# AnnSeidel/genometools

Hardware: AMD Instinct MI355X
Metric: Gbp/s ESA build (suf+lcp+bwt), 3 Gbp DNA, 1/2/4/8 MI355X; bit-exact vs CPU (higher is better)
Workload: dtype u64; 1 GPU; human-like DNA (2% N, 24 seqs, repeats) n=3000000000 seed=43 -suf -lcp -bwt (BASELINE.json configs[2]); parallelism=1 device, pair_suffixes=341032298, tied_suffixes=390540711, refine_rounds=9, maxbranchdepth=8256

## Files before the change

### genometools_amd/csrc/esa_engine.hip

```cpp
#include <stdarg.h>
#include <stdlib.h>
#include <chrono>
#include <type_traits>
#include <utility>
#include <vector>
#include "../../include/gtamd_esa.h"
#include "esa_prims.h"
#include "esa_devutil.h"
#include "esa_own.h"

static thread_local char g_err[1024] = "";
void gtamd_set_error(const char *fmt, ...) {
  va_list ap;
  va_start(ap, fmt);
  vsnprintf(g_err, sizeof g_err, fmt, ap);
  va_end(ap);
}
extern "C" const char *gtamd_esa_last_error(void) { return g_err; }

extern "C" int gtamd_device_count(void) {
  GTAMD_ABI_BEGIN
  int n = 0;
  if (hipGetDeviceCount(&n) != hipSuccess) return 0;
  return n;
// ... 2443 lines not shown
    const long v = atol(e);
    if (v >= MS_TILE && v <= (long) MSD_BIG_MAX) sw.msd_big_max = (u32) v;
  }
  sw.msd_radix = flag("GTAMD_MSD_RADIX", '1');
  if (const char *e = getenv("GTAMD_MSD_PACK")) sw.msd_pack = atoi(e) != 0;
  if (const char *e = getenv("GTAMD_MSD_PACK_CAP")) {
    const long v = atol(e);
    if (v >= 1024 && v <= (long) MD_CAP) sw.msd_pack_cap = (u32) v;
  }
  if (const char *e = getenv("GTAMD_MSD_BIN_LIMIT")) {
    const long v = atol(e);
    if (v >= 2 && v <= 4096) sw.msd_bin_limit = (u32) v;
  }
  sw.fused_pass0 = !flag("GTAMD_FUSED_PASS0", '0');
  sw.force_wide = flag("GTAMD_FORCE_WIDE", '1');
  sw.no_pairs = flag("GTAMD_NO_PAIRS", '1');
  sw.no_small_groups = flag("GTAMD_NO_SMALL_GROUPS", '1');
  if (const char *e = getenv("GTAMD_APPLY_EARLY")) sw.apply_early = atoi(e);
  if (sw.apply_early < 0 || sw.apply_early > 2) sw.apply_early = 0;
  if (const char *e = getenv("GTAMD_APPLY_WGS")) {
    const long v = atol(e);
    if (v >= 64 && v <= (1 << 22)) sw.apply_wgs = (u64) v;
    sw.apply_wgs_given = true;
  }
  if (const char *e = getenv("GTAMD_RANK_WINDOW_BITS")) {
    const int v = atoi(e);
    if (v >= 2 && v <= RW_BITS) sw.rank_window_bits = v;
  }
  sw.rank_all_windows = flag("GTAMD_RANK_ALL_WINDOWS", '1');
  sw.win_filter_global = flag("GTAMD_WIN_FILTER_LDS", '0');
  if (const char *e = getenv("GTAMD_PAIR_CHUNK")) {
    const int v = atoi(e);
    if (v >= 4 && v <= 1024) sw.pair_chunk = v;
  }
  if (const char *e = getenv("GTAMD_ROUND_STRIDE")) {
    const int v = atoi(e);
    if (v >= RT_STRIDE_MIN && v <= RT_TILE) sw.round_stride = (u32) v;
  }
  sw.debug = getenv("GTAMD_DEBUG") != nullptr;
  return sw;
}

struct gtamd_esa_ctx {
  int device = 0;
  u32 sigma = 0;
  int bits = 0;
  u64 max_n = 0, n = 0, N = 0;
  int readmode = 0;
  Stream st, st2;
  Event ev_sorted, ev_emitted, ev_applied;
  DevBuf tb_own, sp_own;
  Text text = {};
  bool have_text = false;
  DevBuf k0, k1, v0, v1;
  DevBuf isa_tmp;
  DevBuf rws;
  DevBuf msd;
  DevBuf suf, lcp, bwt;
  DevBuf tiebits, tiebits2;
  DevBuf arena;
  DevBuf arena_p;
  DevBuf xrecv;
  DevBuf winbuf;
  DevBuf lcpfull_buf;
  DevBuf partws;
  DevBuf posw;
  Dev<u64> llv;
  u64 llv_pairs = 0;
  Dev<u32> bck;
  u64 bck_codes = 0, bck_special = 0, bck_dist = 0;
  Dev<Stats> d_stats;
  Pinned<Stats> h_stats;
  Pinned<u32> h_counts;
  Pinned<u32> h_hist;
  u32 user_prefixlength = 0;
  u32 part = 0, numparts = 1;
  gtamd_allgather_fn comm_allgather = nullptr;
  gtamd_alltoallv_fn comm_alltoallv = nullptr;
  void (*comm_abort)(void *) = nullptr;
  void *comm_abort_user = nullptr;
  void *comm_user = nullptr;
  u64 NL = 0, index_offset = 0;
  Dev<u32> d_parthist;
  Dev<u8> d_owner;
  Dev<u32> d_counts;
  u32 want = 0;
  bool ran = false;
  gtamd_esa_stats stats = {};
  gtamd_esa_timing timing = {};
  u64 alloc_bytes = 0;
  float alloc_ms = 0;
  Event ev[8];
  Event ev_scatter[2 * 16];
};

enum TimingEvent {
  EV_START,
  EV_KEYS,
  EV_SORTED,
  EV_TIEBITS,
  EV_REFINE_BEGIN,
  EV_REFINE_END,
  EV_DONE
};

static int ensure_buf(gtamd_esa_ctx *c, DevBuf &b, u64 bytes, const char *what) {
// ... 104 lines not shown
  GTAMD_ABI_BEGIN
  if (c == nullptr) { gtamd_set_error("null context"); return -1; }
  c->comm_allgather = ag;
  c->comm_alltoallv = a2a;
  c->comm_user = user;
  c->comm_abort = nullptr;
  c->comm_abort_user = nullptr;
  return 0;
  GTAMD_ABI_END(-1)
}

extern "C" int gtamd_esa_set_comm_abort(gtamd_esa_ctx *c, void (*abort_fn)(void *), void *user) {
  GTAMD_ABI_BEGIN
  if (c == nullptr) { gtamd_set_error("null context"); return -1; }
  c->comm_abort = abort_fn;
  c->comm_abort_user = user;
  return 0;
  GTAMD_ABI_END(-1)
}

extern "C" int gtamd_esa_set_prefixlength(gtamd_esa_ctx *c, uint32_t k) {
  GTAMD_ABI_BEGIN
  if (c == nullptr) { gtamd_set_error("null context"); return -1; }
  const u32 maxk = c->bits == 2 ? (u32) KeyLayout<2>::KEY_SYMS : (u32) KeyLayout<5>::KEY_SYMS;
  if (k > maxk) {
    gtamd_set_error("prefix length %u is too large: the maximal prefix length "
                    "for this engine is %u", k, maxk);
    return -1;
  }
  c->user_prefixlength = k;
  return 0;
  GTAMD_ABI_END(-1)
}

extern "C" int gtamd_esa_set_readmode(gtamd_esa_ctx *c, int readmode) {
  GTAMD_ABI_BEGIN
  if (c == nullptr) { gtamd_set_error("null context"); return -1; }
  if (readmode < 0 || readmode > 3) {
    gtamd_set_error("invalid readmode %d (0 forward, 1 reverse, 2 complement, "
                    "3 reverse complement)", readmode);
    return -1;
  }
  if (readmode >= 2 && c->sigma != 4) {
    gtamd_set_error("readmode %s is only defined for DNA alphabets",
                    readmode == 2 ? "cpl" : "rcl");
    return -1;
  }
  c->readmode = readmode;
  c->have_text = false;
  return 0;
  GTAMD_ABI_END(-1)
}

static int set_n(gtamd_esa_ctx *c, u64 n) {
  if (n > c->max_n) {
    gtamd_set_error("sequence length %llu exceeds the context capacity %llu",
                    (unsigned long long) n, (unsigned long long) c->max_n);
    return -1;
  }
  c->n = n;
  c->N = n + 1;
  c->ran = false;
  return 0;
}

extern "C" int gtamd_esa_set_sequence_bytes(gtamd_esa_ctx *c,
                                            const uint8_t *enc, uint64_t n,
                                            int is_device) {
  GTAMD_ABI_BEGIN
  if (c == nullptr) { gtamd_set_error("null context"); return -1; }
  TRY(set_n(c, n));
  HIP_TRY(hipSetDevice(c->device));
  const u64 spw = c->bits == 2 ? 32 : 12;
  const u64 nw_tb = div_up(c->N, spw), nw_sp = div_up(c->N, 64);
  TRY(ensure_buf(c, c->tb_own, (nw_tb + 2) * 8, "the packed sequence"));
  TRY(ensure_buf(c, c->sp_own, (nw_sp + 2) * 8, "the special bitmap"));
  const u8 *d_enc = enc;
  Dev<u8> staged;
  if (!is_device && n > 0) {
    HIP_TRY(staged.alloc(n));
    HIP_TRY(hipMemcpyAsync(staged, enc, n, hipMemcpyHostToDevice, c->st));
    d_enc = staged;
  }
  u64 *tb = c->tb_own.as<u64>(), *sp = c->sp_own.as<u64>();
  const int rev = c->readmode & 1, cpl = c->readmode >> 1;
  if (c->bits == 2)
    k_pack_symbols<2><<<(u32) div_up(nw_tb, 256), 256, 0, c->st>>>(d_enc, n, tb, nw_tb, rev, cpl);
  else
    k_pack_symbols<5><<<(u32) div_up(nw_tb, 256), 256, 0, c->st>>>(d_enc, n, tb, nw_tb, rev, cpl);
  HIP_TRY(hipGetLastError());
  k_pack_specials<<<(u32) div_up(nw_sp, 256), 256, 0, c->st>>>(d_enc, n, sp, nw_sp, rev);
  HIP_TRY(hipGetLastError());
  HIP_TRY(hipStreamSynchronize(c->st));
  c->text.tb = tb; c->text.sp = sp; c->text.n = n;
  c->text.nw_tb = nw_tb; c->text.nw_sp = nw_sp;
  c->have_text = true;
  return 0;
  GTAMD_ABI_END(-1)
}

extern "C" int gtamd_esa_set_sequence_packed(gtamd_esa_ctx *c,
                                             const uint64_t *twobit,
                                             const uint64_t *specialbits,
                                             uint64_t n) {
  GTAMD_ABI_BEGIN
  if (c == nullptr) { gtamd_set_error("null context"); return -1; }
  if (c->bits != 2) {
    gtamd_set_error("packed input is defined for the 2-bit DNA layout only");
    return -1;
  }
  if (c->readmode != 0) {
    gtamd_set_error("packed input is read in place: readmode %d cannot be applied "
                    "(hand the sequence in as bytes)", c->readmode);
    return -1;
  }
  TRY(set_n(c, n));
  c->text.tb = twobit; c->text.sp = specialbits; c->text.n = n;
  c->text.nw_tb = div_up(n, 32); c->text.nw_sp = div_up(n + 1, 64);
  c->have_text = true;
  return 0;
  GTAMD_ABI_END(-1)
}

static int fetch_stats(gtamd_esa_ctx *c) {
  HIP_TRY(hipMemcpyAsync(c->h_stats, c->d_stats, sizeof(Stats),
                         hipMemcpyDeviceToHost, c->st));
  HIP_TRY(hipStreamSynchronize(c->st));
  return 0;
}

static int bits_for(u64 maxvalue) {
  int b = 1;
  while (b < 64 && (maxvalue >> b) != 0) b++;
  return b;
}

struct Bump {
  u8 *base;
  u64 off;
  template <typename T> T *take(u64 count) {
    off = (off + 255) & ~255ull;
    T *p = base != nullptr ? reinterpret_cast<T *>(base + off) : nullptr;
    off += count * sizeof(T);
    return p;
  }
};

static int comm_allgather(gtamd_esa_ctx *c, int failed, const void *send, void *recv,
                          u32 bytes) {
  const u32 R = c->numparts;
  if (R == 1 && c->comm_allgather == nullptr) {
    if (bytes) memcpy(recv, send, bytes);
    return failed ? -1 : 0;
  }
  std::vector<u8> mine(8 + (size_t) bytes), all((size_t) R * (8 + bytes));
  const u64 status = failed ? 1 : 0;
  memcpy(mine.data(), &status, 8);
  if (bytes) memcpy(mine.data() + 8, send, bytes);
  const auto t0 = std::chrono::steady_clock::now();
  const int rc = c->comm_allgather(c->comm_user, mine.data(), all.data(), 8 + bytes);
  c->timing.comm_ms += std::chrono::duration<float, std::milli>(
                           std::chrono::steady_clock::now() - t0).count();
  c->timing.comm_calls++;
  if (rc != 0) {
    gtamd_set_error("allgather callback failed");
    return -1;
  }
  int bad = -1;
  for (u32 r = 0; r < R; r++) {
    u64 s;
    memcpy(&s, all.data() + (size_t) r * (8 + bytes), 8);
// ... 78 lines not shown
    k_bck_count<BITS><<<(u32) div_up(NL, 256), 256, 0, st>>>(
        skey, NL, k, c->sigma, c->bck, c->bck + codes + 1,
        c->bck + codes + 1 + special, c->text, spos);
    HIP_TRY(hipGetLastError());
  }
  u32 *ws = c->rws.as<u32>();
  Dev<u32> own;
  if (scan_workspace_words(codes + 1) * 4 > c->rws.bytes) {
    HIP_TRY(own.alloc(scan_workspace_words(codes + 1) * 4));
    ws = own;
  }
  TRY(scan_u32(SCAN_SUM, c->bck, c->bck, codes + 1, false, ws, st));
  c->bck_codes = codes; c->bck_special = special; c->bck_dist = dist;
  return 0;
}

static u64 rws_words_for(u64 cap) {
  return radix_workspace_words(cap) + 10 * (div_up(cap, 64) + 64) +
         scan_workspace_words(div_up(cap, 64)) + 64;
}
static int ensure_workspace(gtamd_esa_ctx *c, u64 cap, u32 want, bool dist) {
  const u64 pad = cap + 8;
  TRY(ensure_buf(c, c->k0, pad * 8, "sort keys"));
  TRY(ensure_buf(c, c->k1, pad * 8, "sort keys"));
  TRY(ensure_buf(c, c->v0, pad * 4, "sort values"));
  TRY(ensure_buf(c, c->v1, pad * 4, "sort values"));
  TRY(ensure_buf(c, c->rws, rws_words_for(cap) * 4, "the radix workspace"));
  TRY(ensure_buf(c, c->tiebits, (div_up(cap, 64) + 2) * 8, "the tie bitmap"));
  if (want & GTAMD_WANT_SUF) TRY(ensure_buf(c, c->suf, pad * 8, "the suffix table"));
  if (want & GTAMD_WANT_LCP) TRY(ensure_buf(c, c->lcp, pad, "the lcp table"));
  if (want & GTAMD_WANT_BWT) TRY(ensure_buf(c, c->bwt, pad, "the bwt table"));
  if (dist) TRY(ensure_buf(c, c->isa_tmp, pad * 8, "the exchange scratch"));
  return 0;
}

static int msd_cbits_max(u64 N) {
  const int c = bits_for(N > 1 ? N - 1 : 1) - 24;
  return c < 0 ? 0 : (c > 8 ? 8 : c);
}
static int msd_choose_cbits(u64 N, int cmax, const float *penalty) {
  int best = cmax;
  float best_cost = 0.0f;
  for (int k = 1; k >= 0; k--) {
    const int c = cmax - 2 + k;
    if (c < 6) continue;
    const float gain = k == 1 ? 0.17f : 0.57f;
    const float cost = (penalty[k] - penalty[2]) / (float) N - gain;
    if (cost < best_cost) { best = c; best_cost = cost; }
  }
  return best;
}
struct MsdWs {
  u32 *hist, *scanws, *tcnt, *tfirst, *dtcnt, *dtfirst, *startA, *startB, *F, *scan2, *counters,
      *biglist, *giantlist, *crowdlist, *bndA;
  MsTile *desc;
  MdTile *dtiles;
  u64 *firstkey, *lastkey;
  u32 rows, tilesB_ub, tilesC_ub, tilesD_ub;
  u64 nf;
};
static u64 msd_carve(u64 N, int cb, u8 *base, MsdWs *w) {
  const u32 ntA = (u32) div_up(N, MS_TILE);
  w->tilesB_ub = ntA + 256;
  w->tilesC_ub = ntA + MSD_PARENTS;
  w->tilesD_ub = (u32) (2 * div_up(N, MS_TILE)) + MSD_PARENTS + 8;
  w->rows = w->tilesC_ub + 2;
  w->nf = (u64) MSD_PARENTS << cb;
  Bump b;
  b.base = base;
  b.off = 0;
  w->hist = b.take<u32>((u64) w->rows * 256);
  w->scanws = b.take<u32>(radix_rows_workspace_words(w->rows));
  w->desc = b.take<MsTile>(w->tilesC_ub);
  w->tcnt = b.take<u32>(MSD_PARENTS + 8);
  w->tfirst = b.take<u32>(MSD_PARENTS + 8);
  w->dtcnt = b.take<u32>(MSD_PARENTS + 8);
  w->dtfirst = b.take<u32>(MSD_PARENTS + 8);
  w->startA = b.take<u32>(256 + 8);
  w->bndA = b.take<u32>(256 * MSD_BLOCKS);
  w->startB = b.take<u32>(MSD_PARENTS + 8);
  w->F = b.take<u32>(w->nf + 8);
  w->scan2 = b.take<u32>(scan_workspace_words(w->nf + 1) + 64);
  w->counters = b.take<u32>(16);
  w->dtiles = b.take<MdTile>(w->tilesD_ub);
  w->firstkey = b.take<u64>(w->tilesD_ub);
  w->lastkey = b.take<u64>(w->tilesD_ub);
  w->biglist = b.take<u32>(w->tilesD_ub);
  w->crowdlist = b.take<u32>(w->tilesD_ub);
  w->giantlist = b.take<u32>((u64) (N / MS_TILE) + 8);
  return b.off + 256;
}

static int msd_level_prepare(gtamd_esa_ctx *c, const MsdWs &w, const u32 *pstart, u32 np, int cb,
                             u32 tiles_ub, const u32 *kin, const u64 *ein, u32 *cstart) {
  hipStream_t st = c->st;
  k_msd_tilecount<<<(np + 1 + 255) / 256, 256, 0, st>>>(pstart, 0, np, (u32) MS_TILE, w.tcnt);
  HIP_TRY(hipGetLastError());
  TRY(scan_u32(SCAN_SUM, w.tcnt, w.tfirst, (u64) np + 1, false, w.scan2, st));
  k_msd_tiledesc<<<(tiles_ub + 255) / 256, 256, 0, st>>>(pstart, w.tfirst, np, tiles_ub, w.desc);
  HIP_TRY(hipGetLastError());
  if (ein != nullptr)
    k_msd_hist_lvl<u64><<<tiles_ub + 1, MS_THREADS, 0, st>>>(ein, w.desc, tiles_ub, 32 - cb, w.hist);
  else
    k_msd_hist_lvl<u32><<<tiles_ub + 1, MS_THREADS, 0, st>>>(kin, w.desc, tiles_ub, 32 - cb, w.hist);
  HIP_TRY(hipGetLastError());
  TRY(radix_scan_tile_rows(w.hist, tiles_ub + 1, w.scanws, st));
  const u64 nchild = (u64) np << cb;
  k_msd_tot<<<(u32) div_up(nchild + 1, 256), 256, 0, st>>>(w.hist, w.tfirst, np, cb, cstart);
  HIP_TRY(hipGetLastError());
  TRY(scan_u32(SCAN_SUM, cstart, cstart, nchild + 1, false, w.scan2, st));
  return 0;
}

struct MsdPartSrc {
  const u64 *ck;
  const u32 *cp32;
  u64 index_offset;
  const unsigned long long *prev_key;
  int has_prev;
};
template <int FMT>
static int msd_sort_emit(gtamd_esa_ctx *c, const Switches &sw, u32 want, u32 prefixlength, u64 N,
                         u64 density_n, const MsdPartSrc *src, u32 **sa_out,
                         u64 **fkey, u32 **fval, u64 *local_entries) {
  hipStream_t st = c->st;
  const int cmax = msd_cbits_max(density_n);
  int cb = sw.msd_cbits >= 0 ? sw.msd_cbits : cmax;
  MsdWs w;
  const u64 bytes = msd_carve(N, cb > cmax ? cb : cmax, nullptr, &w);
  TRY(ensure_buf(c, c->msd, bytes, "the tables of the first sort"));
  (void) msd_carve(N, cb > cmax ? cb : cmax, c->msd.as<u8>(), &w);
  const u32 ntA = (u32) div_up(N, MS_TILE);
  const u32 last_valid = (u32) (N - (u64) (ntA - 1) * MS_TILE);
  const u64 pad = N + 8;
  u32 *ka = c->k0.as<u32>(), *pa = c->v0.as<u32>();
  u32 *kb = c->k1.as<u32>(), *pb = c->v1.as<u32>();
  u8 *xa = c->k1.as<u8>() + pad * 4;
  u64 *ea = c->k0.as<u64>();
  const bool wide = src == nullptr;
  const int lbits = msd_block_bits(N);
  if (src != nullptr)
    k_msd_hist_a_keys<<<ntA, MS_THREADS, 0, st>>>(src->ck, N, w.hist);
  else if (FMT == 1)
    k_msd_hist_a5<<<ntA, MS_THREADS, 0, st>>>(c->text, N, w.hist);
  else
    k_msd_hist_a<<<ntA, MS_THREADS, 0, st>>>(c->text, N, w.hist);
  HIP_TRY(hipGetLastError());
  TRY(radix_scan_tile_rows(w.hist, ntA, w.scanws, st));
  k_msd_starts_a<<<wide ? MSD_BLOCKS : 1, 256, 0, st>>>(w.hist, (u32) N, ntA, lbits, w.startA,
                                                         wide ? w.bndA : nullptr);
  HIP_TRY(hipGetLastError());
  if (src != nullptr)
    k_msd_scatter_a<1><<<((ntA + 7u) >> 3) * 8u, MS_THREADS, 0, st>>>(
        c->text, N, last_valid, w.hist, ntA, src->ck, src->cp32, ka, xa, pa, nullptr);
  else if (FMT == 1)
    k_msd_scatter_a<2><<<((ntA + 7u) >> 3) * 8u, MS_THREADS, 0, st>>>(
        c->text, N, last_valid, w.hist, ntA, nullptr, nullptr, nullptr, nullptr, nullptr, ea);
  else
    k_msd_scatter_a<0><<<((ntA + 7u) >> 3) * 8u, MS_THREADS, 0, st>>>(
        c->text, N, last_valid, w.hist, ntA, nullptr, nullptr, nullptr, nullptr, nullptr, ea);
  HIP_TRY(hipGetLastError());
  HIP_TRY(hipEventRecord(c->ev[EV_KEYS], st));
  TRY(msd_level_prepare(c, w, w.startA, 256, 8, w.tilesB_ub, ka, wide ? ea : nullptr, w.startB));
  if (wide)
    k_msd_scatter_lvl<1, true><<<((w.tilesB_ub + 7u) >> 3) * 8u, MS_THREADS, 0, st>>>(
        nullptr, nullptr, nullptr, ea, w.bndA, lbits, w.desc, w.tilesB_ub, w.hist, w.tfirst,
        w.startB, 8, 24, kb, pb);
  else
    k_msd_scatter_lvl<1, false><<<((w.tilesB_ub + 7u) >> 3) * 8u, MS_THREADS, 0, st>>>(
        ka, xa, pa, nullptr, nullptr, 0, w.desc, w.tilesB_ub, w.hist, w.tfirst, w.startB, 8, 24,
        kb, pb);
  HIP_TRY(hipGetLastError());
  if (sw.msd_cbits < 0 && cmax >= 1) {
    float *d_exp = reinterpret_cast<float *>(w.counters);
    float *h_exp = c->h_counts.as<float>();
    HIP_TRY(hipMemsetAsync(d_exp, 0, 16, st));
    k_msd_skew<<<MSD_PARENTS / 256, 256, 0, st>>>(w.startB, cmax, d_exp);
    HIP_TRY(hipGetLastError());
    HIP_TRY(hipMemcpyAsync(h_exp, d_exp, 12, hipMemcpyDeviceToHost, st));
    HIP_TRY(hipStreamSynchronize(st));
    cb = msd_choose_cbits(N, cmax, h_exp);
  }
  w.nf = (u64) MSD_PARENTS << cb;
  u32 *kf = kb, *pf = pb, *ko = ka, *po = pa;
  const u32 *F = w.startB;
  if (cb > 0) {
    TRY(msd_level_prepare(c, w, w.startB, MSD_PARENTS, cb, w.tilesC_ub, kb, nullptr, w.F));
    F = w.F;
    kf = ka; pf = pa; ko = kb; po = pb;
  }
  HIP_TRY(hipMemsetAsync(w.counters, 0, 64, st));
  const u32 pack_cap = sw.msd_pack_cap;
  const bool packed = sw.msd_pack;
  if (packed) {
    k_msd_pack<false><<<(MSD_PARENTS + 1 + 255) / 256, 256, 0, st>>>(F, cb, nullptr, pack_cap, w.dtcnt, nullptr,
                                                                nullptr, nullptr, nullptr, 0);
    HIP_TRY(hipGetLastError());
    TRY(scan_u32(SCAN_SUM, w.dtcnt, w.dtfirst, (u64) MSD_PARENTS + 1, false, w.scan2, st));
    k_msd_pack<true><<<(MSD_PARENTS + 1 + 255) / 256, 256, 0, st>>>(F, cb, w.dtfirst, pack_cap, nullptr, w.dtiles,
                                                               w.biglist, w.giantlist, w.counters,
                                                               sw.msd_big_max);
    HIP_TRY(hipGetLastError());
// ... 2 lines not shown
                                                               w.dtcnt);
  HIP_TRY(hipGetLastError());
  TRY(scan_u32(SCAN_SUM, w.dtcnt, w.dtfirst, (u64) MSD_PARENTS + 1, false, w.scan2, st));
  k_msd_dtiles<<<(w.tilesD_ub + 255) / 256, 256, 0, st>>>(F, cb, w.dtfirst, w.tilesD_ub, w.dtiles,
                                                        w.biglist, w.giantlist, w.crowdlist,
                                                        w.counters, sw.msd_big_max);
  HIP_TRY(hipGetLastError());
  }
  u32 *hc = c->h_counts;
  HIP_TRY(hipMemcpyAsync(hc, w.counters, 16, hipMemcpyDeviceToHost, st));
  HIP_TRY(hipMemcpyAsync(hc + 4, w.dtfirst + MSD_PARENTS, 4, hipMemcpyDeviceToHost, st));
  HIP_TRY(hipStreamSynchronize(st));
  const u32 nbig = hc[0], maxrun = hc[1], nbigentries = hc[2], ngiant = hc[3], ntD = hc[4];
  char dpre[32] = "";
  if (src != nullptr) snprintf(dpre, sizeof dpre, "part %u: ", c->part);
  if (sw.debug) {
    fprintf(stderr, "gtamd: %smsd sort: %d bits at level C, %u runs, %u big (largest %u, %u entries "
            "in all), %u giant\n", dpre, cb, ntD, nbig, maxrun, nbigentries, ngiant);
    std::vector<MdTile> dt(ntD);
    if (ntD > 0)
      HIP_TRY(hipMemcpy(dt.data(), w.dtiles, (size_t) ntD * sizeof(MdTile), hipMemcpyDeviceToHost));
    u32 largest = 0;
    for (const MdTile &d : dt) largest = d.end - d.begin > largest ? d.end - d.begin : largest;
    fprintf(stderr, "gtamd: %smsd level D: packed=%d pack_cap=%u tiles=%u largest=%u\n", dpre,
            (int) packed, pack_cap, ntD, largest);
  }
  std::vector<MdTile> giants(ngiant);
  std::vector<u32> giant_t(ngiant);
  if (ngiant > 0) {
    HIP_TRY(hipMemcpy(giant_t.data(), w.giantlist, (size_t) ngiant * 4, hipMemcpyDeviceToHost));
    for (u32 i = 0; i < ngiant; i++)
      HIP_TRY(hipMemcpy(&giants[i], w.dtiles + giant_t[i], sizeof(MdTile), hipMemcpyDeviceToHost));
  }
  if (cb > 0) {
    k_msd_scatter_lvl<2, false><<<((w.tilesC_ub + 7u) >> 3) * 8u, MS_THREADS, 0, st>>>(
        kb, nullptr, pb, nullptr, nullptr, 0, w.desc, w.tilesC_ub, w.hist, w.tfirst, w.F, cb,
        32 - cb, ka, pa);
    HIP_TRY(hipGetLastError());
  }
  MsdOut o;
  o.suf = (want & GTAMD_WANT_SUF) ? c->suf.as<u64>() : nullptr;
  o.lcp = (want & GTAMD_WANT_LCP) ? c->lcp.as<u8>() : nullptr;
  o.bwt = (want & GTAMD_WANT_BWT) ? c->bwt.as<u8>() : nullptr;
  o.sa = pf;
  o.tiebits = c->tiebits.as<u64>();
  o.firstkey = w.firstkey;
  o.lastkey = w.lastkey;
  o.stats = c->d_stats;
  o.prefixlength = prefixlength;
  o.index_offset = src != nullptr ? src->index_offset : 0;
  o.val_is_index = src != nullptr && src->cp32 == nullptr;
  if (o.val_is_index) o.suf = nullptr;
  HIP_TRY(hipMemsetAsync(o.tiebits, 0, (div_up(N, 64) + 2) * 8, st));
  if (ntD > 0) {
    HIP_TRY(hipEventRecord(c->ev_scatter[0], st));
    const int force_radix = sw.msd_radix ? 1 : 0;
    k_msd_local<FMT><<<stride_grid(ntD), MS_THREADS, 0, st>>>(kf, pf, w.dtiles, ntD, cb,
                                                        force_radix, sw.msd_bin_limit,
                                                        w.crowdlist, w.counters, o);
    HIP_TRY(hipEventRecord(c->ev_scatter[1], st));
    HIP_TRY(hipGetLastError());
    k_msd_local_radix<FMT><<<ntD < 2048u ? ntD : 2048u, MS_THREADS, 0, st>>>(kf, pf, w.dtiles,
                                                                        w.crowdlist, w.counters,
                                                                        cb, o);
    HIP_TRY(hipGetLastError());
    if (sw.debug) {
      HIP_TRY(hipMemcpyAsync(hc + 6, w.counters + 4, 4, hipMemcpyDeviceToHost, st));
      HIP_TRY(hipStreamSynchronize(st));
      fprintf(stderr, "gtamd: %smsd local: radix_runs=%u force_radix=%d bin_limit=%u\n", dpre, hc[6],
              force_radix, sw.msd_bin_limit);
    }
  }
  if (nbig > 0) {
    k_msd_big<FMT><<<nbig < 2048u ? nbig : 2048u, MS_THREADS, 0, st>>>(kf, pf, ko, po, w.dtiles,
                                                                w.biglist, w.counters, cb, o);
    HIP_TRY(hipGetLastError());
  }
  for (u32 i = 0; i < ngiant; i++) {
    const MdTile g = giants[i];
    const u64 cnt = g.end - g.begin;
    const int shifts[4] = {FMT == 1 ? 8 : 3, FMT == 1 ? 14 : 11, FMT == 1 ? 20 : 19, FMT == 1 ? 26 : 27};
    const int widths[4] = {FMT == 1 ? 6 : 8, FMT == 1 ? 6 : 8, FMT == 1 ? 6 : 8, FMT == 1 ? 6 : 5};
    int nev = 0;
    TRY(radix_sort_pairs<u32, u32>(kf + g.begin, pf + g.begin, ko + g.begin, po + g.begin, cnt,
                                   shifts, widths, 4, c->rws.as<u32>(), st, nullptr, &nev));
    k_msd_emit_run<FMT><<<(u32) div_up(cnt, MS_TILE), MS_THREADS, 0, st>>>(kf, pf, giant_t[i], g.begin,
                                                                     (u32) cnt, g.s16, o);
    HIP_TRY(hipGetLastError());
  }
  if (ntD > 0) {
    k_msd_seams<FMT><<<(ntD + 255) / 256, 256, 0, st>>>(w.dtiles, ntD, src != nullptr ? src->prev_key : nullptr,
                                                   src != nullptr ? src->has_prev : 0, o);
    HIP_TRY(hipGetLastError());
  }
  *sa_out = pf;
  *fkey = reinterpret_cast<u64 *>(ko);
  *fval = po;
  *local_entries = N - nbigentries;
  c->stats.msd_big_entries = nbigentries;
  return 0;
}

static int passes_for(int from, int to, int *ps, int *pw) {
  int cnt = 0;
  for (int b = from; b < to; b += 8) {
    ps[cnt] = b;
    pw[cnt] = to - b < 8 ? to - b : 8;
    cnt++;
  }
  return cnt;
}

template <typename T>
static std::vector<u32> range_cuts(const T *bins, u32 R) {
  u64 nsamp = 0;
  for (int b = 0; b < PART_BINS; b++) nsamp += bins[b];
  std::vector<u32> cut(R + 1);
  cut[0] = 0;
  cut[R] = PART_BINS;
  u64 run = 0;
  u32 b = 0;
  for (u32 r = 1; r < R; r++) {
    const u64 target = (u64) (((unsigned __int128) nsamp * r) / R);
    while (b < (u32) PART_BINS && run < target) run += bins[b++];
    cut[r] = b;
  }
  return cut;
}

enum Reduce { RED_SUM, RED_AND, RED_OR, RED_MAX };
static int allgather_word(gtamd_esa_ctx *c, int failed, Reduce op, u64 *word) {
  std::vector<u64> all(c->numparts);
  TRY(comm_allgather(c, failed, word, all.data(), 8));
  u64 v = all[0];
  for (u32 r = 1; r < c->numparts; r++)
    switch (op) {
      case RED_SUM: v += all[r]; break;
      case RED_AND: v &= all[r]; break;
      case RED_OR: v |= all[r]; break;
      case RED_MAX: v = all[r] > v ? all[r] : v; break;
    }
  *word = v;
  return 0;
}

static void set_slice_error(u64 NL) {
  gtamd_set_error("slice of %llu entries exceeds the 32-bit index range of one "
                  "part: use more parts", (unsigned long long) NL);
}

struct WinFilterTies {
// ... 1613 lines not shown
```

### genometools_amd/csrc/esa_msd.h

```cpp
#pragma once
#include "esa_msd_blocks.h"

constexpr int MS_TILE = 4096;
constexpr int MS_THREADS = 512;
constexpr int MS_WAVES = MS_THREADS / 64;
constexpr int MS_ITEMS = MS_TILE / MS_THREADS;
constexpr int MS_WCHUNK = MS_ITEMS * 64;
constexpr int MS_PAD = 520;
constexpr u32 MSD_PARENTS = 65536;
constexpr u32 MSD_STRIDE = 3328;
constexpr int MD_ITEMS = 8;
constexpr u32 MD_CAP = MD_ITEMS * MS_THREADS;
constexpr u32 MSD_BIG_MAX = 1u << 19;

struct MsTile {
  u32 start;
  u32 segvalid;
};
struct MdTile {
  u32 begin, end;
  u32 s16;
  u32 pad;
};
struct MsdOut {
  u64 *suf;
  u8 *lcp;
  u8 *bwt;
  u32 *sa;
  u64 *tiebits;
  u64 *firstkey, *lastkey;
  Stats *stats;
  u32 prefixlength;
  u64 index_offset;
  u32 val_is_index;
};
struct MsdAcc {
  unsigned long long sum, ties;
  u32 mx;
};

__device__ __forceinline__ u32 ms_xcd_tile(u32 b, u32 ntiles) {
  const u32 per = (ntiles + 7u) >> 3;
  return (b & 7u) * per + (b >> 3);
}

template <int FMT> struct MsdFmt;
template <> struct MsdFmt<0> {
  static constexpr int PB = 3;
  static constexpr u32 KSYMS = 20;
};
template <> struct MsdFmt<1> {
  static constexpr int PB = 8;
  static constexpr u32 KSYMS = 8;
// ... 141 lines not shown
    u32 sx = (u32) ((int) (d << (31 - b)) >> 31);
    asm volatile("" : "+v"(sx));
    const u64 bal = __ballot(sx != 0);
    mlo = __builtin_amdgcn_bitop3_b32(mlo, (u32) bal, sx, 0x90);
    mhi = __builtin_amdgcn_bitop3_b32(mhi, (u32) (bal >> 32), sx, 0x90);
  }
  intra = __builtin_amdgcn_mbcnt_hi(mhi, __builtin_amdgcn_mbcnt_lo(mlo, 0u));
  group = (u32) __popc(mlo) + (u32) __popc(mhi);
}

typedef __attribute__((address_space(3))) volatile u16 ms_vu16;

__device__ __forceinline__ void lds_barrier() {
  asm volatile("s_waitcnt lgkmcnt(0)\n\ts_barrier" ::: "memory");
}
__device__ __forceinline__ u32 ms_scan_excl(u32 v, u32 *lds8) {
  const int lane = threadIdx.x & 63, w = threadIdx.x >> 6;
  const u32 inc = wave_scan_incl<SCAN_SUM>(v);
  if (lane == 63) lds8[w] = inc;
  lds_barrier();
  u32 carry = 0;
#pragma unroll
  for (int i = 0; i < MS_WAVES; i++) {
    const u32 x = lds8[i];
    if (i < w) carry += x;
  }
  lds_barrier();
  return carry + (inc - v);
}

__global__ __launch_bounds__(MS_THREADS) void k_msd_hist_a5(Text t, u64 N, u32 *__restrict__ hist) {
  __shared__ u32 h[MS_WAVES][256];
  const int tid = threadIdx.x, w = tid >> 6;
  for (int i = tid; i < MS_WAVES * 256; i += MS_THREADS) (&h[0][0])[i] = 0;
  __syncthreads();
  const u64 p0 = (u64) blockIdx.x * MS_TILE + (u64) tid * KP_PER;
  if (p0 < N) {
    const int npos = N - p0 < KP_PER ? (int) (N - p0) : KP_PER;
    u64 key[KP_PER];
    p5_keys8(t, p0, key);
#pragma unroll
    for (int g = 0; g < KP_PER; g++)
      if (g < npos) atomicAdd(&h[w][(u32) (key[g] >> 56)], 1u);
  }
  __syncthreads();
  if (tid < 256) {
    u32 c = 0;
#pragma unroll
    for (int i = 0; i < MS_WAVES; i++) c += h[i][tid];
    hist[(u64) blockIdx.x * 256 + tid] = c;
  }
}

__global__ __launch_bounds__(MS_THREADS) void k_msd_hist_a(Text t, u64 N,
                                                           u32 *__restrict__ hist) {
  __shared__ u32 h[MS_WAVES][256];
  const int tid = threadIdx.x, w = tid >> 6;
  for (int i = tid; i < MS_WAVES * 256; i += MS_THREADS) (&h[0][0])[i] = 0;
  __syncthreads();
  const u64 p0 = (u64) blockIdx.x * MS_TILE + (u64) tid * KP_PER;
  if (p0 < N) {
    const int npos = N - p0 < KP_PER ? (int) (N - p0) : KP_PER;
    u64 key[KP_PER];
    dna_keys8(t, p0, key);
#pragma unroll
    for (int g = 0; g < KP_PER; g++)
      if (g < npos) atomicAdd(&h[w][(u32) (key[g] >> 56)], 1u);
  }
  __syncthreads();
  if (tid < 256) {
    u32 c = 0;
#pragma unroll
    for (int i = 0; i < MS_WAVES; i++) c += h[i][tid];
    hist[(u64) blockIdx.x * 256 + tid] = c;
  }
}

struct DnaWin {
  u64 a_hi, a_lo;
  u64 S;
  u32 pay0;
};
__device__ __forceinline__ DnaWin dna_win(const Text &t, u64 p0) {
  using P = Pay<2>;
  DnaWin r;
  const u64 w = p0 >> 5;
  const int o = (int) (p0 & 31) * 2;
  const u64 hi = tb_word(t, w), lo = tb_word(t, w + 1);
  r.a_hi = o ? (hi << o) | (lo >> (64 - o)) : hi;
  r.a_lo = lo << o;
  const u64 sw = p0 >> 6;
  const int so = (int) (p0 & 63);
  const u64 s0 = sp_word(t, sw), s1 = sp_word(t, sw + 1);
  r.S = so ? (s0 >> so) | (s1 << (64 - so)) : s0;
  if (p0 == 0) {
    r.pay0 = P::UNDEF;
  } else {
    const u32 c = o ? (u32) (hi >> (64 - o)) & 3u : (u32) tb_word(t, w - 1) & 3u;
    const bool sp = c < 2u && (so ? (s0 >> (so - 1)) & 1ull : sp_word(t, sw - 1) >> 63);
    r.pay0 = sp ? ((c & 1u) ? P::SEP : P::WILD) : c;
  }
  return r;
}
__device__ __forceinline__ DnaWin dna_win_from(const Text &t, u64 p0, u64 hi, u64 lo, u64 s0, u64 s1) {
  using P = Pay<2>;
  DnaWin r;
  const u64 w = p0 >> 5;
  const int o = (int) (p0 & 31) * 2;
  r.a_hi = o ? (hi << o) | (lo >> (64 - o)) : hi;
  r.a_lo = lo << o;
  const u64 sw = p0 >> 6;
  const int so = (int) (p0 & 63);
  r.S = so ? (s0 >> so) | (s1 << (64 - so)) : s0;
  if (p0 == 0) {
    r.pay0 = P::UNDEF;
  } else {
    const u32 c = o ? (u32) (hi >> (64 - o)) & 3u : (u32) tb_word(t, w - 1) & 3u;
    const bool sp = c < 2u && (so ? (s0 >> (so - 1)) & 1ull : sp_word(t, sw - 1) >> 63);
    r.pay0 = sp ? ((c & 1u) ? P::SEP : P::WILD) : c;
  }
// ... 164 lines not shown
  __syncthreads();
  const u64 base = (u64) blockIdx.x * MS_TILE;
#pragma unroll
  for (int j = 0; j < MS_ITEMS; j++) {
    const u64 e = base + (u64) j * MS_THREADS + tid;
    if (e < M) atomicAdd(&h[w][(u32) (ck[e] >> 56)], 1u);
  }
  __syncthreads();
  if (tid < 256) {
    u32 c = 0;
#pragma unroll
    for (int i = 0; i < MS_WAVES; i++) c += h[i][tid];
    hist[(u64) blockIdx.x * 256 + tid] = c;
  }
}

__global__ __launch_bounds__(256) void k_part_positions(const u32 *__restrict__ idx,
                                                        const u64 *__restrict__ cp, u64 M,
                                                        u64 index_offset, u64 *__restrict__ sa64,
                                                        u64 *__restrict__ suf, Stats *stats) {
  const u64 i = (u64) blockIdx.x * 256 + threadIdx.x;
  if (i >= M) return;
  const u64 p = cp[idx[i]];
  sa64[i] = p;
  if (suf != nullptr) suf[i] = p;
  if (p == 0) stats->longest = index_offset + i;
}

__global__ __launch_bounds__(256) void k_msd_starts_a(const u32 *__restrict__ scanned, u32 N,
                                                      u32 ntiles, int L, u32 *__restrict__ start,
                                                      u32 *__restrict__ bnd) {
  const u32 d = threadIdx.x, k = blockIdx.x;
  if (k == 0) {
    start[d] = scanned[d];
    if (d == 0) start[256] = N;
  }
  if (bnd != nullptr) {
    const u32 t = k << (L - 12);
    const u32 end = d < 255u ? scanned[d + 1] : N;
    bnd[d * MSD_BLOCKS + k] = t < ntiles ? scanned[(u64) t * 256 + d] : end;
  }
}

template <int SRC>
__global__ __launch_bounds__(MS_THREADS) void k_msd_scatter_a(
    Text t, u64 N, u32 last_valid, const u32 *__restrict__ scanned, u32 ntiles,
    const u64 *__restrict__ ck, const u32 *__restrict__ cp32,
    u32 *__restrict__ k1out, u8 *__restrict__ xout, u32 *__restrict__ pout,
    u64 *__restrict__ eout) {
  __shared__ u64 s_t[5120];
  __shared__ u16 s_cnt_mem[MS_WAVES * 256];
  __shared__ u32 s_obase[256];
  __shared__ u32 s_scan[MS_WAVES];
  static_assert(KP_PER * MS_PAD <= 5120 && MS_TILE * 10 <= 5120 * 8 && MS_TILE * 9 <= 5120 * 8,
                "staging fits");
  const int tid = threadIdx.x, lane = tid & 63, w = tid >> 6;
  const u32 tile = ms_xcd_tile(blockIdx.x, ntiles);
  if (tile >= ntiles) return;
  const u64 tile_base = (u64) tile * MS_TILE;
  const u32 valid = tile + 1u == ntiles ? last_valid : (u32) MS_TILE;
  for (int i = tid; i < MS_WAVES * 256 / 2; i += MS_THREADS)
    reinterpret_cast<u32 *>(s_cnt_mem)[i] = 0;
  u32 gbase = 0;
  if (tid < 256) gbase = scanned[(u64) tile * 256 + tid];
  constexpr bool FROMKEYS = SRC == 1;
  u64 key[MS_ITEMS];
  u32 rk[MS_ITEMS], val[MS_ITEMS];
  if (FROMKEYS) {
#pragma unroll
    for (int j = 0; j < MS_ITEMS; j++) {
      const u32 e = (u32) w * MS_WCHUNK + (u32) j * 64 + lane;
      key[j] = e < valid ? ck[tile_base + e] : ~0ull;
      val[j] = (e < valid && cp32 != nullptr) ? cp32[tile_base + e] : (u32) tile_base + e;
    }
  } else {
  {
    u64 key8[KP_PER];
    const u64 p0 = tile_base + (u64) tid * KP_PER;
    if (p0 < N) {
      if (SRC == 2) p5_keys8(t, p0, key8);
      else dna_keys8(t, p0, key8);
    } else {
#pragma unroll
      for (int g = 0; g < KP_PER; g++) key8[g] = ~0ull;
    }
#pragma unroll
    for (int g = 0; g < KP_PER; g++) s_t[g * MS_PAD + tid] = key8[g];
  }
  __syncthreads();
#pragma unroll
  for (int j = 0; j < MS_ITEMS; j++) {
    const u32 e = (u32) w * MS_WCHUNK + (u32) j * 64 + lane;
    key[j] = s_t[(e & 7u) * MS_PAD + (e >> 3)];
  }
  }
  __syncthreads();
  ms_vu16 *cnt_w = (ms_vu16 *) s_cnt_mem + w * 256;
#pragma unroll
  for (int j = 0; j < MS_ITEMS; j++) {
    const u32 e = (u32) w * MS_WCHUNK + (u32) j * 64 + lane;
    const u32 d = e < valid ? (u32) (key[j] >> 56) : 255u;
    u32 intra, group;
    ms_match<8>(d, intra, group);
    const u32 old = cnt_w[d];
    if (intra == 0) cnt_w[d] = (u16) (old + group);
    rk[j] = ((old + intra) << 8) | d;
  }
  __syncthreads();
  {
    ms_vu16 *s_cnt = (ms_vu16 *) s_cnt_mem;
    u32 c[MS_WAVES];
    u32 tot = 0;
    if (tid < 256) {
#pragma unroll
      for (int i = 0; i < MS_WAVES; i++) {
        c[i] = s_cnt[i * 256 + tid];
        tot += c[i];
      }
    }
    u32 all;
    u32 dbase = block_scan_excl<SCAN_SUM, MS_THREADS>(tot, &all, s_scan);
    if (tid < 256) {
      s_obase[tid] = gbase - dbase;
#pragma unroll
      for (int i = 0; i < MS_WAVES; i++) {
        s_cnt[i * 256 + tid] = (u16) dbase;
        dbase += c[i];
      }
    }
  }
  __syncthreads();
  if (!FROMKEYS) {
    u8 *s_d = reinterpret_cast<u8 *>(s_t + MS_TILE);
#pragma unroll
    for (int j = 0; j < MS_ITEMS; j++) {
      const u32 e = (u32) w * MS_WCHUNK + (u32) j * 64 + lane;
      const u32 d = rk[j] & 255u;
      const u32 pos = (u32) cnt_w[d] + (rk[j] >> 8);
      const u32 x = SRC == 2 ? (u32) key[j] & 63u
                             : (((u32) (key[j] >> 19) & 31u) << 3) | ((u32) key[j] & 7u);
      s_t[pos] = ((key[j] >> 24) << 32) | ((u64) x << 24) | (u64) (((u32) tile_base + e) & 0xFFFFFFu);
      s_d[pos] = (u8) d;
    }
    __syncthreads();
#pragma unroll
    for (int j = 0; j < MS_ITEMS; j++) {
      const u32 e = (u32) j * MS_THREADS + tid;
      if (e < valid) eout[s_obase[s_d[e]] + e] = s_t[e];
    }
    return;
  }
  u32 *s_k1 = reinterpret_cast<u32 *>(s_t);
  u32 *s_p = s_k1 + MS_TILE;
  u8 *s_x = reinterpret_cast<u8 *>(s_p + MS_TILE);
  u8 *s_d = s_x + MS_TILE;
#pragma unroll
  for (int j = 0; j < MS_ITEMS; j++) {
    const u32 e = (u32) w * MS_WCHUNK + (u32) j * 64 + lane;
    const u32 d = rk[j] & 255u;
    const u32 pos = (u32) cnt_w[d] + (rk[j] >> 8);
    s_k1[pos] = (u32) (key[j] >> 24);
    s_p[pos] = FROMKEYS ? val[j] : (u32) tile_base + e;
    s_x[pos] = SRC == 2 ? (u8) ((u32) key[j] & 63u)
                        : (u8) ((((u32) (key[j] >> 19) & 31u) << 3) | ((u32) key[j] & 7u));
    s_d[pos] = (u8) d;
  }
  __syncthreads();
#pragma unroll
  for (int j = 0; j < MS_ITEMS; j++) {
    const u32 e = (u32) j * MS_THREADS + tid;
    if (e < valid) {
      const u32 g = s_obase[s_d[e]] + e;
      k1out[g] = s_k1[e];
      pout[g] = s_p[e];
      xout[g] = s_x[e];
    }
  }
}

__global__ __launch_bounds__(256) void k_msd_tilecount(const u32 *__restrict__ pstart, int sh,
                                                       u32 np, u32 per, u32 *__restrict__ cnt) {
  const u32 s = blockIdx.x * 256u + threadIdx.x;
  if (s > np) return;
  if (s == np) { cnt[s] = 0; return; }
  const u32 size = pstart[(u64) (s + 1) << sh] - pstart[(u64) s << sh];
  cnt[s] = (size + per - 1u) / per;
}

__device__ __forceinline__ u32 ms_parent_of(const u32 *__restrict__ tfirst, u32 np, u32 t) {
  u32 lo = 0, hi = np;
  while (hi - lo > 1) {
    const u32 mid = (lo + hi) >> 1;
    if (tfirst[mid] <= t) lo = mid; else hi = mid;
  }
  return lo;
}

__global__ __launch_bounds__(256) void k_msd_tiledesc(const u32 *__restrict__ pstart,
                                                      const u32 *__restrict__ tfirst, u32 np,
                                                      u32 tiles_ub, MsTile *__restrict__ desc) {
  const u32 t = blockIdx.x * 256u + threadIdx.x;
  if (t >= tiles_ub) return;
  MsTile d;
  d.start = 0;
// ... 901 lines not shown
      const u32 valid = cnt - c0 < (u32) MS_TILE ? cnt - c0 : (u32) MS_TILE;
#pragma unroll
      for (int j = 0; j < MS_ITEMS; j++) {
        const u32 e = (u32) j * MS_THREADS + tid;
        if (e < valid) {
          s_key[e] = sk[c0 + e] - base;
          s_val[e] = sp[c0 + e];
        }
      }
      __syncthreads();
      if (tid == 0) {
        if (c0 == 0) o.firstkey[t] = msd_full<FMT>(td.s16, s_key[0] + base);
        if (c0 + valid == cnt) o.lastkey[t] = msd_full<FMT>(td.s16, s_key[valid - 1] + base);
      }
      const u32 lastk = s_key[valid - 1] + base;
      msd_emit<FMT>(s_key, s_val, valid, (u64) td.begin + c0, base, c0 > 0, prevkey, td.s16, o, s_bits, acc);
      prevkey = lastk;
    }
  }
  msd_acc_flush(acc, o.stats);
}

template <int FMT>
__global__ __launch_bounds__(MS_THREADS) void k_msd_emit_run(
    const u32 *__restrict__ kin, const u32 *__restrict__ pin, u32 t, u32 begin, u32 cnt, u32 s16,
    MsdOut o) {
  __shared__ u32 s_key[MS_TILE];
  __shared__ u32 s_val[MS_TILE];
  __shared__ u32 s_bits[(MS_TILE + 128) / 32];
  const int tid = threadIdx.x;
  MsdAcc acc;
  acc.sum = acc.ties = 0;
  acc.mx = 0;
  const u32 c0 = blockIdx.x * (u32) MS_TILE;
  const u32 valid = cnt - c0 < (u32) MS_TILE ? cnt - c0 : (u32) MS_TILE;
#pragma unroll
  for (int j = 0; j < MS_ITEMS; j++) {
    const u32 e = (u32) j * MS_THREADS + tid;
    if (e < valid) {
      s_key[e] = kin[(u64) begin + c0 + e];
      s_val[e] = pin[(u64) begin + c0 + e];
    }
  }
  __syncthreads();
  if (tid == 0) {
    if (c0 == 0) o.firstkey[t] = msd_full<FMT>(s16, s_key[0]);
    if (c0 + valid == cnt) o.lastkey[t] = msd_full<FMT>(s16, s_key[valid - 1]);
  }
  const u32 prevkey = c0 > 0 ? kin[(u64) begin + c0 - 1] : 0u;
  msd_emit<FMT>(s_key, s_val, valid, (u64) begin + c0, 0u, c0 > 0, prevkey, s16, o, s_bits, acc);
  msd_acc_flush(acc, o.stats);
}

template <int FMT>
__global__ __launch_bounds__(256) void k_msd_seams(const MdTile *__restrict__ tiles, u32 ntiles,
                                                   const unsigned long long *__restrict__ prev_key_p,
                                                   int has_prev, MsdOut o) {
  using K = Key<2>;
  const u32 t = blockIdx.x * 256u + threadIdx.x;
  MsdAcc acc;
  acc.sum = acc.ties = 0;
  acc.mx = 0;
  if (t < ntiles) {
    const MdTile td = tiles[t];
    if (td.end > td.begin && (td.begin > 0 || has_prev)) {
      u64 a = has_prev ? (u64) *prev_key_p : 0ull;
      if (td.begin > 0) {
        u32 u = t - 1;
        while (u > 0 && tiles[u].end == tiles[u].begin) u--;
        a = o.lastkey[u];
      }
      const u64 b = o.firstkey[t];
      u32 da, db, m;
      if (FMT == 1) {
        da = p5_letters(a >> 8); db = p5_letters(b >> 8);
        m = p5_common(a >> 8, b >> 8);
      } else {
        da = K::letters(a); db = K::letters(b);
        const u64 x = (a ^ b) >> K::LOW_BITS;
        m = x ? (u32) (__clzll((long long) x) - K::LOW_BITS) / 2u : (u32) K::SYMS;
      }
      u32 l = m < da ? m : da;
      l = l < db ? l : db;
      if (o.lcp != nullptr) o.lcp[td.begin] = (u8) l;
      acc.mx = l;
      if (db >= o.prefixlength) acc.sum = l;
    }
  }
  msd_acc_flush(acc, o.stats);
}
```

Before: 26.30 Gbp/s.

## Drop special-position suffixes from MSD sort and emit them in a separate tail pass

Counts special (N/separator) positions once when the sequence is set, then excludes those suffixes from the MSD histogram and scatter in the 2-bit wide path. A dedicated tail kernel writes them directly at the end of the suffix array in position order, with zero LCP and their BWT symbol. This is meant to avoid sorting and refining the ~2% special suffixes, which share maximal keys and tie. In exchange it adds a popcount pre-pass with a host sync at sequence setup, a branchier ranking path in tiles that contain specials, and correctness risk in the output offsets and the placement of the longest suffix.

Result: slower. 25.74 Gbp/s (-2.1%).

```diff
diff --git a/genometools_amd/csrc/esa_engine.hip b/genometools_amd/csrc/esa_engine.hip
--- a/genometools_amd/csrc/esa_engine.hip
+++ b/genometools_amd/csrc/esa_engine.hip
@@ -2519,6 +2519,7 @@
   DevBuf tb_own, sp_own;
   Text text = {};
   bool have_text = false;
+  u64 nspecial = 0;
   DevBuf k0, k1, v0, v1;
   DevBuf isa_tmp;
   DevBuf rws;
@@ -2729,6 +2730,22 @@
   GTAMD_ABI_END(-1)
 }
 
+static int count_specials(gtamd_esa_ctx *c) {
+  c->nspecial = 0;
+  if (c->bits != 2) return 0;
+  unsigned long long *acc = c->d_counts.as<unsigned long long>();
+  unsigned long long *hacc = c->h_counts.as<unsigned long long>();
+  const u64 ntiles = div_up(c->N, MS_TILE);
+  HIP_TRY(hipMemsetAsync(acc, 0, 8, c->st));
+  k_msd_tail_count<<<(u32) div_up(ntiles, MS_WAVES), MS_THREADS, 0, c->st>>>(c->text, c->N, (u32) ntiles,
+                                                                       nullptr, acc);
+  HIP_TRY(hipGetLastError());
+  HIP_TRY(hipMemcpyAsync(hacc, acc, 8, hipMemcpyDeviceToHost, c->st));
+  HIP_TRY(hipStreamSynchronize(c->st));
+  c->nspecial = hacc[0];
+  return 0;
+}
+
 static int set_n(gtamd_esa_ctx *c, u64 n) {
   if (n > c->max_n) {
     gtamd_set_error("sequence length %llu exceeds the context capacity %llu",
@@ -2771,6 +2788,7 @@
   HIP_TRY(hipStreamSynchronize(c->st));
   c->text.tb = tb; c->text.sp = sp; c->text.n = n;
   c->text.nw_tb = nw_tb; c->text.nw_sp = nw_sp;
+  TRY(count_specials(c));
   c->have_text = true;
   return 0;
   GTAMD_ABI_END(-1)
@@ -2794,6 +2812,8 @@
   TRY(set_n(c, n));
   c->text.tb = twobit; c->text.sp = specialbits; c->text.n = n;
   c->text.nw_tb = div_up(n, 32); c->text.nw_sp = div_up(n + 1, 64);
+  HIP_TRY(hipSetDevice(c->device));
+  TRY(count_specials(c));
   c->have_text = true;
   return 0;
   GTAMD_ABI_END(-1)
@@ -2978,7 +2998,7 @@
 }
 struct MsdWs {
   u32 *hist, *scanws, *tcnt, *tfirst, *dtcnt, *dtfirst, *startA, *startB, *F, *scan2, *counters,
-      *biglist, *giantlist, *crowdlist, *bndA;
+      *biglist, *giantlist, *crowdlist, *bndA, *tailcnt, *tailscan;
   MsTile *desc;
   MdTile *dtiles;
   u64 *firstkey, *lastkey;
@@ -3014,6 +3034,8 @@
   w->biglist = b.take<u32>(w->tilesD_ub);
   w->crowdlist = b.take<u32>(w->tilesD_ub);
   w->giantlist = b.take<u32>((u64) (N / MS_TILE) + 8);
+  w->tailcnt = b.take<u32>((u64) ntA + 8);
+  w->tailscan = b.take<u32>(scan_workspace_words(ntA) + 64);
   return b.off + 256;
 }
 
@@ -3065,6 +3087,13 @@
   u64 *ea = c->k0.as<u64>();
   const bool wide = src == nullptr;
   const int lbits = msd_block_bits(N);
+  const bool tail = wide && FMT == 0;
+  if (tail && (c->nspecial == 0 || c->nspecial > N)) {
+    gtamd_set_error("%llu special positions in a table of %llu entries", (unsigned long long) c->nspecial,
+                    (unsigned long long) N);
+    return -1;
+  }
+  const u64 Ns = tail ? N - c->nspecial : N;
   if (src != nullptr)
     k_msd_hist_a_keys<<<ntA, MS_THREADS, 0, st>>>(src->ck, N, w.hist);
   else if (FMT == 1)
@@ -3073,7 +3102,7 @@
     k_msd_hist_a<<<ntA, MS_THREADS, 0, st>>>(c->text, N, w.hist);
   HIP_TRY(hipGetLastError());
   TRY(radix_scan_tile_rows(w.hist, ntA, w.scanws, st));
-  k_msd_starts_a<<<wide ? MSD_BLOCKS : 1, 256, 0, st>>>(w.hist, (u32) N, ntA, lbits, w.startA,
+  k_msd_starts_a<<<wide ? MSD_BLOCKS : 1, 256, 0, st>>>(w.hist, (u32) Ns, ntA, lbits, w.startA,
                                                          wide ? w.bndA : nullptr);
   HIP_TRY(hipGetLastError());
   if (src != nullptr)
@@ -3182,6 +3211,13 @@
   o.val_is_index = src != nullptr && src->cp32 == nullptr;
   if (o.val_is_index) o.suf = nullptr;
   HIP_TRY(hipMemsetAsync(o.tiebits, 0, (div_up(N, 64) + 2) * 8, st));
+  if (tail) {
+    k_msd_tail_count<<<(u32) div_up(ntA, MS_WAVES), MS_THREADS, 0, st>>>(c->text, N, ntA, w.tailcnt, nullptr);
+    HIP_TRY(hipGetLastError());
+    TRY(scan_u32(SCAN_SUM, w.tailcnt, w.tailcnt, ntA, false, w.tailscan, st));
+    k_msd_tail<<<ntA, MS_THREADS, 0, st>>>(c->text, N, Ns, w.tailcnt, o);
+    HIP_TRY(hipGetLastError());
+  }
   if (ntD > 0) {
     HIP_TRY(hipEventRecord(c->ev_scatter[0], st));
     const int force_radix = sw.msd_radix ? 1 : 0;
@@ -3226,7 +3262,7 @@
   *sa_out = pf;
   *fkey = reinterpret_cast<u64 *>(ko);
   *fval = po;
-  *local_entries = N - nbigentries;
+  *local_entries = Ns - nbigentries;
   c->stats.msd_big_entries = nbigentries;
   return 0;
 }
diff --git a/genometools_amd/csrc/esa_msd.h b/genometools_amd/csrc/esa_msd.h
--- a/genometools_amd/csrc/esa_msd.h
+++ b/genometools_amd/csrc/esa_msd.h
@@ -1,4 +1,5 @@
 #pragma once
+#include <type_traits>
 #include "esa_msd_blocks.h"
 
 constexpr int MS_TILE = 4096;
@@ -246,6 +247,10 @@
   }
 }
 
+__device__ __forceinline__ u32 dna_special8(const Text &t, u64 p0, int npos) {
+  return (u32) (sp_word(t, p0 >> 6) >> (p0 & 63)) & ((1u << npos) - 1u);
+}
+
 __global__ __launch_bounds__(MS_THREADS) void k_msd_hist_a(Text t, u64 N,
                                                            u32 *__restrict__ hist) {
   __shared__ u32 h[MS_WAVES][256];
@@ -257,9 +262,10 @@
     const int npos = N - p0 < KP_PER ? (int) (N - p0) : KP_PER;
     u64 key[KP_PER];
     dna_keys8(t, p0, key);
+    const u32 keep = ~dna_special8(t, p0, npos) & ((1u << npos) - 1u);
 #pragma unroll
     for (int g = 0; g < KP_PER; g++)
-      if (g < npos) atomicAdd(&h[w][(u32) (key[g] >> 56)], 1u);
+      if ((keep >> g) & 1u) atomicAdd(&h[w][(u32) (key[g] >> 56)], 1u);
   }
   __syncthreads();
   if (tid < 256) {
@@ -530,6 +536,7 @@
   __shared__ u16 s_cnt_mem[MS_WAVES * 256];
   __shared__ u32 s_obase[256];
   __shared__ u32 s_scan[MS_WAVES];
+  __shared__ u32 s_drops;
   static_assert(KP_PER * MS_PAD <= 5120 && MS_TILE * 10 <= 5120 * 8 && MS_TILE * 9 <= 5120 * 8,
                 "staging fits");
   const int tid = threadIdx.x, lane = tid & 63, w = tid >> 6;
@@ -539,6 +546,7 @@
   const u32 valid = tile + 1u == ntiles ? last_valid : (u32) MS_TILE;
   for (int i = tid; i < MS_WAVES * 256 / 2; i += MS_THREADS)
     reinterpret_cast<u32 *>(s_cnt_mem)[i] = 0;
+  if (tid == 0) s_drops = 0;
   u32 gbase = 0;
   if (tid < 256) gbase = scanned[(u64) tile * 256 + tid];
   constexpr bool FROMKEYS = SRC == 1;
@@ -552,12 +560,14 @@
       val[j] = (e < valid && cp32 != nullptr) ? cp32[tile_base + e] : (u32) tile_base + e;
     }
   } else {
+  u32 mine = 0;
   {
     u64 key8[KP_PER];
     const u64 p0 = tile_base + (u64) tid * KP_PER;
     if (p0 < N) {
       if (SRC == 2) p5_keys8(t, p0, key8);
       else dna_keys8(t, p0, key8);
+      if (SRC == 0) mine = dna_special8(t, p0, N - p0 < KP_PER ? (int) (N - p0) : KP_PER);
     } else {
 #pragma unroll
       for (int g = 0; g < KP_PER; g++) key8[g] = ~0ull;
@@ -566,6 +576,7 @@
     for (int g = 0; g < KP_PER; g++) s_t[g * MS_PAD + tid] = key8[g];
   }
   __syncthreads();
+  if (mine) s_drops = 1;
 #pragma unroll
   for (int j = 0; j < MS_ITEMS; j++) {
     const u32 e = (u32) w * MS_WCHUNK + (u32) j * 64 + lane;
@@ -574,60 +585,71 @@
   }
   __syncthreads();
   ms_vu16 *cnt_w = (ms_vu16 *) s_cnt_mem + w * 256;
-#pragma unroll
-  for (int j = 0; j < MS_ITEMS; j++) {
-    const u32 e = (u32) w * MS_WCHUNK + (u32) j * 64 + lane;
-    const u32 d = e < valid ? (u32) (key[j] >> 56) : 255u;
-    u32 intra, group;
-    ms_match<8>(d, intra, group);
-    const u32 old = cnt_w[d];
-    if (intra == 0) cnt_w[d] = (u16) (old + group);
-    rk[j] = ((old + intra) << 8) | d;
-  }
-  __syncthreads();
-  {
-    ms_vu16 *s_cnt = (ms_vu16 *) s_cnt_mem;
-    u32 c[MS_WAVES];
-    u32 tot = 0;
-    if (tid < 256) {
-#pragma unroll
-      for (int i = 0; i < MS_WAVES; i++) {
-        c[i] = s_cnt[i * 256 + tid];
-        tot += c[i];
-      }
-    }
-    u32 all;
-    u32 dbase = block_scan_excl<SCAN_SUM, MS_THREADS>(tot, &all, s_scan);
-    if (tid < 256) {
-      s_obase[tid] = gbase - dbase;
-#pragma unroll
-      for (int i = 0; i < MS_WAVES; i++) {
-        s_cnt[i * 256 + tid] = (u16) dbase;
-        dbase += c[i];
-      }
-    }
-  }
-  __syncthreads();
-  if (!FROMKEYS) {
-    u8 *s_d = reinterpret_cast<u8 *>(s_t + MS_TILE);
+  auto rank_and_store = [&](auto with_drops) {
+    constexpr bool DROPS = decltype(with_drops)::value;
+    constexpr u32 DROPPED = ~0u;
 #pragma unroll
     for (int j = 0; j < MS_ITEMS; j++) {
       const u32 e = (u32) w * MS_WCHUNK + (u32) j * 64 + lane;
-      const u32 d = rk[j] & 255u;
-      const u32 pos = (u32) cnt_w[d] + (rk[j] >> 8);
-      const u32 x = SRC == 2 ? (u32) key[j] & 63u
-                             : (((u32) (key[j] >> 19) & 31u) << 3) | ((u32) key[j] & 7u);
-      s_t[pos] = ((key[j] >> 24) << 32) | ((u64) x << 24) | (u64) (((u32) tile_base + e) & 0xFFFFFFu);
-      s_d[pos] = (u8) d;
+      const bool keep = e < valid && !(DROPS && Key<2>::dcode(key[j]) == Key<2>::DMAX);
+      const u32 d = keep ? (u32) (key[j] >> 56) : (DROPS ? 256u : 255u);
+      u32 intra, group;
+      ms_match<DROPS ? 9 : 8>(d, intra, group);
+      const u32 dc = DROPS ? d & 255u : d;
+      const u32 old = cnt_w[dc];
+      if (intra == 0 && (!DROPS || keep)) cnt_w[dc] = (u16) (old + group);
+      rk[j] = (DROPS && !keep) ? DROPPED : ((old + intra) << 8) | d;
     }
     __syncthreads();
-#pragma unroll
-    for (int j = 0; j < MS_ITEMS; j++) {
-      const u32 e = (u32) j * MS_THREADS + tid;
-      if (e < valid) eout[s_obase[s_d[e]] + e] = s_t[e];
-    }
-    return;
-  }
+    u32 nout = valid;
+    {
+      ms_vu16 *s_cnt = (ms_vu16 *) s_cnt_mem;
+      u32 c[MS_WAVES];
+      u32 tot = 0;
+      if (tid < 256) {
+#pragma unroll
+        for (int i = 0; i < MS_WAVES; i++) {
+          c[i] = s_cnt[i * 256 + tid];
+          tot += c[i];
+        }
+      }
+      u32 all;
+      u32 dbase = block_scan_excl<SCAN_SUM, MS_THREADS>(tot, &all, s_scan);
+      if (DROPS) nout = all;
+      if (tid < 256) {
+        s_obase[tid] = gbase - dbase;
+#pragma unroll
+        for (int i = 0; i < MS_WAVES; i++) {
+          s_cnt[i * 256 + tid] = (u16) dbase;
+          dbase += c[i];
+        }
+      }
+    }
+    __syncthreads();
+    if (!FROMKEYS) {
+      u8 *s_d = reinterpret_cast<u8 *>(s_t + MS_TILE);
+#pragma unroll
+      for (int j = 0; j < MS_ITEMS; j++) {
+        const u32 e = (u32) w * MS_WCHUNK + (u32) j * 64 + lane;
+        if (DROPS && rk[j] == DROPPED) continue;
+        const u32 d = rk[j] & 255u;
+        const u32 pos = (u32) cnt_w[d] + (rk[j] >> 8);
+        const u32 x = SRC == 2 ? (u32) key[j] & 63u
+                               : (((u32) (key[j] >> 19) & 31u) << 3) | ((u32) key[j] & 7u);
+        s_t[pos] = ((key[j] >> 24) << 32) | ((u64) x << 24) | (u64) (((u32) tile_base + e) & 0xFFFFFFu);
+        s_d[pos] = (u8) d;
+      }
+      __syncthreads();
+#pragma unroll
+      for (int j = 0; j < MS_ITEMS; j++) {
+        const u32 e = (u32) j * MS_THREADS + tid;
+        if (e < nout) eout[s_obase[s_d[e]] + e] = s_t[e];
+      }
+    }
+  };
+  if (SRC == 0 && uni(s_drops) != 0) rank_and_store(std::true_type());
+  else rank_and_store(std::false_type());
+  if (!FROMKEYS) return;
   u32 *s_k1 = reinterpret_cast<u32 *>(s_t);
   u32 *s_p = s_k1 + MS_TILE;
   u8 *s_x = reinterpret_cast<u8 *>(s_p + MS_TILE);
@@ -1635,6 +1657,85 @@
   msd_acc_flush(acc, o.stats);
 }
 
+__global__ __launch_bounds__(MS_THREADS) void k_msd_tail_count(Text t, u64 N, u32 ntiles,
+                                                               u32 *__restrict__ cnt,
+                                                               unsigned long long *total) {
+  const u32 tile = blockIdx.x * (u32) MS_WAVES + (threadIdx.x >> 6);
+  if (tile >= ntiles) return;
+  const u64 wi = (u64) tile * (MS_TILE / 64) + (threadIdx.x & 63);
+  u64 word = sp_word(t, wi);
+  const u64 base = wi * 64;
+  if (base >= N) word = 0;
+  else if (N - base < 64) word &= (1ull << (N - base)) - 1ull;
+  u32 v = (u32) __popcll(word);
+  for (int d = 32; d >= 1; d >>= 1) v += __shfl_xor(v, d, 64);
+  if ((threadIdx.x & 63) == 0) {
+    if (cnt != nullptr) cnt[tile] = v;
+    if (total != nullptr && v != 0) atomicAdd(total, (unsigned long long) v);
+  }
+}
+
+__global__ __launch_bounds__(MS_THREADS) void k_msd_tail(Text t, u64 N, u64 Ns,
+                                                         const u32 *__restrict__ tfirst,
+                                                         MsdOut o) {
+  __shared__ u32 s_pos[MS_TILE];
+  __shared__ u8 s_bw[MS_TILE];
+  __shared__ u32 s_scan[MS_WAVES];
+  const int tid = threadIdx.x;
+  const u64 p0 = (u64) blockIdx.x * MS_TILE + (u64) tid * KP_PER;
+  u32 mine = 0;
+  if (p0 < N) mine = dna_special8(t, p0, N - p0 < KP_PER ? (int) (N - p0) : KP_PER);
+  u32 cnt;
+  u32 r = block_scan_excl<SCAN_SUM, MS_THREADS>((u32) __popc(mine), &cnt, s_scan);
+  if (cnt == 0) return;
+  if (mine) {
+    u64 key[KP_PER];
+    dna_keys8(t, p0, key);
+#pragma unroll
+    for (int g = 0; g < KP_PER; g++) {
+      if ((mine >> g) & 1u) {
+        s_pos[r] = (u32) p0 + (u32) g;
+        s_bw[r] = Pay<2>::to_bwt((u32) key[g] & 7u);
+        r++;
+      }
+    }
+  }
+  __syncthreads();
+  const u64 gbeg = Ns + (u64) tfirst[blockIdx.x];
+  if (gbeg + cnt > N) return;
+  const u32 mis = (u32) (gbeg & 3);
+  const u32 nquads = (cnt + mis + 3u) >> 2;
+  const u64 gq = gbeg - mis;
+  for (u32 q = tid; q < nquads; q += MS_THREADS) {
+    const int i0 = (int) (4u * q) - (int) mis;
+    const u64 g0 = gq + 4ull * q;
+    if (i0 >= 0 && i0 + 4 <= (int) cnt) {
+      const u32 a = s_pos[i0], b = s_pos[i0 + 1], c = s_pos[i0 + 2], d = s_pos[i0 + 3];
+      if (o.suf != nullptr) {
+        *reinterpret_cast<ulonglong2 *>(o.suf + g0) = make_ulonglong2(a, b);
+        *reinterpret_cast<ulonglong2 *>(o.suf + g0 + 2) = make_ulonglong2(c, d);
+      }
+      *reinterpret_cast<uint4 *>(o.sa + g0) = make_uint4(a, b, c, d);
+      if (o.lcp != nullptr) *reinterpret_cast<u32 *>(o.lcp + g0) = 0u;
+      if (o.bwt != nullptr)
+        *reinterpret_cast<u32 *>(o.bwt + g0) = (u32) s_bw[i0] | ((u32) s_bw[i0 + 1] << 8) |
+                                               ((u32) s_bw[i0 + 2] << 16) | ((u32) s_bw[i0 + 3] << 24);
+      if (a == 0) o.stats->longest = g0;
+    } else {
+      for (int c = 0; c < 4; c++) {
+        const int i = i0 + c;
+        if (i < 0 || i >= (int) cnt) continue;
+        const u32 p = s_pos[i];
+        if (o.suf != nullptr) o.suf[g0 + c] = p;
+        o.sa[g0 + c] = p;
+        if (o.lcp != nullptr) o.lcp[g0 + c] = 0;
+        if (o.bwt != nullptr) o.bwt[g0 + c] = s_bw[i];
+        if (p == 0) o.stats->longest = g0 + (u64) c;
+      }
+    }
+  }
+}
+
 template <int FMT>
 __global__ __launch_bounds__(256) void k_msd_seams(const MdTile *__restrict__ tiles, u32 ntiles,
                                                    const unsigned long long *__restrict__ prev_key_p,
```
